# klasmodin/quflow

Hardware: AMD Instinct MI355X
Metric: isospectral timesteps/sec at N=1024 (1 GPU) + ensemble steps/sec at 1/2/4/8 GPUs (higher is better)
Workload: dtype f64

## Files before the change

### quflow_amd/csrc/api_context.hip

```cpp
#include <cmath>
#include <cstdarg>
#include <cstdio>
#include <cstdlib>
#include <cstring>
#include <limits>
#include <chrono>

#include "qf_api.h"

static thread_local char g_err[512] = "";

void qf_set_error(const char *fmt, ...)
{
    va_list ap;
    va_start(ap, fmt);
    vsnprintf(g_err, sizeof(g_err), fmt, ap);
    va_end(ap);
}

extern "C" {

int qf_version(void) { return QF_VERSION; }

int qf_device_info(int device, char *buf, int n)
// ... 93 lines not shown
    }
    QF_HIP(hipSetDevice(device));
    qf_ctx *ctx = new qf_ctx();
    ctx->N = N;
    ctx->device = device;
    if (const char *g = getenv("QUFLOW_HIP_GEMM")) {
        ctx->gemm_i8_allowed = (g[0] == 'i');
        if (g[0] == 'i' && strstr(g, "x6")) ctx->oz_digits = 6;
        if (g[0] == 'i' && strstr(g, "x65")) ctx->oz_digits2 = 5;
        if (g[0] == 'i' && strchr(g, 'h')) ctx->gemm_i8_hybrid = true;
        if (g[0] == 'i' && strchr(g, 'f') && !ctx->gemm_i8_hybrid) ctx->gemm_i8_first = true;
        if (g[0] == 'a') {
            ctx->gemm_i8_allowed = true;
            ctx->oz_digits = 6;
            ctx->oz_digits2 = 5;
            ctx->gemm_i8_min_n = 1024;
        }
    }
    if (const char *g = getenv("QUFLOW_HIP_GEMM2")) ctx->gemm_tri_allowed = !(g[0] == 'f');
    if (const char *g = getenv("QUFLOW_HIP_FUSED")) ctx->fused_allowed = !(g[0] == '0');
    if (const char *g = getenv("QUFLOW_HIP_I8_MIN_N")) ctx->gemm_i8_min_n = atoi(g);
    if (const char *g = getenv("QUFLOW_HIP_TRI_MIN_N")) ctx->gemm_tri_min_n = atoi(g);
    if (const char *g = getenv("QUFLOW_HIP_DEFER")) ctx->defer_allowed = !(g[0] == '0');
    if (getenv("QUFLOW_HIP_DEBUG"))
        if (const char *g = getenv("QUFLOW_HIP_DEBUG_DROP_FLAG")) ctx->debug_drop = atoi(g);
    if (const char *g = getenv("QUFLOW_HIP_FACTOR_CACHE_MB")) ctx->factor_budget_bytes = (size_t)(atoi(g) > 0 ? atoi(g) : 1) << 20;
    const size_t NN = (size_t)N * N;
    const size_t mbytes = NN * sizeof(cplx);
    int rc = QF_OK;
    auto fail = [&](int code) {
        qf_ctx_destroy(ctx);
        return code;
    };
#define QF_CREATE_HIP(call)                                                                   \
    do {                                                                                      \
        hipError_t _e = (call);                                                               \
        if (_e != hipSuccess) {                                                               \
            qf_set_error("%s failed: %s", #call, hipGetErrorString(_e));                     \
            return fail(QF_ERR_HIP);                                                          \
        }                                                                                     \
    } while (0)
    QF_CREATE_HIP(hipStreamCreateWithFlags(&ctx->stream, hipStreamNonBlocking));
    cplx **mats[] = {&ctx->W, &ctx->dW[0], &ctx->dW[1], &ctx->Whalf, &ctx->Phalf, &ctx->PW, &ctx->stage};
    for (cplx **m : mats) {
        QF_CREATE_HIP(hipMalloc((void **)m, mbytes));
        QF_CREATE_HIP(hipMemsetAsync(*m, 0, mbytes, ctx->stream));
// ... 226 lines not shown
{
    QF_TRY(check_ctx(ctx));
    QF_HIP(hipEventRecord(ctx->timer_start, ctx->stream));
    return QF_OK;
}

int qf_timer_stop(qf_ctx *ctx, double *elapsed_ms)
{
    QF_TRY(check_ctx(ctx));
    QF_HIP(hipEventRecord(ctx->timer_stop, ctx->stream));
    QF_HIP(hipEventSynchronize(ctx->timer_stop));
    float ms = 0.f;
    QF_HIP(hipEventElapsedTime(&ms, ctx->timer_start, ctx->timer_stop));
    if (elapsed_ms) *elapsed_ms = (double)ms;
    return QF_OK;
}

int qf_download_buffer(qf_ctx *ctx, int which, void *host)
{
    QF_TRY(check_ctx(ctx));
    const cplx *src = nullptr;
    switch (which) {
        case QF_BUF_W: src = ctx->W; break;
        case QF_BUF_DW: src = ctx->dW[ctx->dw_cur]; break;
        case QF_BUF_WHALF: src = ctx->Whalf; break;
        case QF_BUF_PHALF: src = ctx->Phalf; break;
        case QF_BUF_PW: src = ctx->PW; break;
        default:
            qf_set_error("qf_download_buffer: unknown buffer %d", which);
            return QF_ERR_INVALID;
    }
    if (!host) {
        qf_set_error("qf_download_buffer: null host pointer");
        return QF_ERR_INVALID;
    }
    QF_HIP(hipMemcpyAsync(host, src, (size_t)ctx->N * ctx->N * sizeof(cplx), hipMemcpyDeviceToHost, ctx->stream));
    QF_HIP(hipStreamSynchronize(ctx->stream));
    return QF_OK;
}

int qf_debug_modulus(qf_ctx *ctx, int n, const double *er_host, const double *ei_host, double *out_modulus_host,
                     double *out_sqrt_host)
{
    QF_TRY(check_ctx(ctx));
    if (n < 1 || (size_t)n > (size_t)ctx->N * ctx->N || !er_host || !ei_host || !out_modulus_host || !out_sqrt_host) {
        qf_set_error("qf_debug_modulus: bad arguments (n=%d)", n);
        return QF_ERR_INVALID;
// ... 14 lines not shown
```

### quflow_amd/csrc/api_isomp.hip

```cpp
#include <cmath>
#include <cstdarg>
#include <cstdio>
#include <cstdlib>
#include <cstring>
#include <limits>
#include <chrono>
#include <type_traits>
#include <utility>

#include "qf_api.h"

namespace {

#ifndef QF_RUN_AHEAD
#define QF_RUN_AHEAD 3
#endif

template <class S> constexpr bool is_c64 = std::is_same<S, qf_c64>::value;

template <class S> S *ws(qf_ctx *ctx)
{
    if constexpr (is_c64<S>) return ctx->c64;
    else return ctx;
}
// ... 87 lines not shown
    ctx->gemm_i8 = want_i8 && skew;
    ctx->gemm_tri32 = want_tri32 && skew && (!ctx->gemm_i8 || ctx->gemm_i8_first);
    if (ctx->gemm_tri32) QF_TRY(tri32_alloc(ctx));
    return QF_OK;
}

int select_second_product_c64(qf_ctx *ctx)
{
    qf_c64 *f = ctx->c64;
    f->tri = false;
    if (f->tri_allowed && ctx->gemm_tri_allowed && (qf_c64_tile(ctx) == 32 || ctx->N % 64 == 0) && ctx->N >= 64) {
        QF_TRY(check_skew(ctx, f));
        if (f->w_skew_known) {
            QF_TRY(qf_c64_tri_alloc(ctx));
            f->tri = true;
        }
    }
    return QF_OK;
}

bool triangle_product(const qf_ctx *ctx) { return (ctx->gemm_tri || ctx->gemm_tri32) && (!ctx->gemm_i8 || ctx->gemm_i8_first); }
bool triangle_product(const qf_c64 *f) { return f->tri; }

template <class S> int begin_increment(qf_ctx *ctx, S *w, bool carry)
{
    const size_t mbytes = (size_t)ctx->N * ctx->N * sizeof(*w->W);
    if (carry) {
        if (w->dw_cur != 0)
            QF_HIP(hipMemcpyAsync(w->dW[0], w->dW[w->dw_cur], mbytes, hipMemcpyDeviceToDevice, ctx->stream));
        QF_TRY(qf_launch_lincomb(ctx, 1, w->W, 1, w->dW[0], 0, w->Whalf));
    } else {
        QF_HIP(hipMemsetAsync(w->dW[0], 0, mbytes, ctx->stream));
        QF_HIP(hipMemcpyAsync(w->Whalf, w->W, mbytes, hipMemcpyDeviceToDevice, ctx->stream));
    }
    return QF_OK;
}

template <class S> int enqueue_iterations(qf_ctx *ctx, int step, int first, int count, double vareps)
{
    S *w = ws<S>(ctx);
    for (int i = first; i < first + count; ++i) {
        qf_guard g;
        g.state = ctx->state;
        g.step = step;
        g.iter = i;
        {
            prof_scope p(ctx, QF_KERNEL_POISSON);
            QF_TRY(launch_solve(ctx, w->Whalf, w->Phalf, vareps, g));
        }
        {
            prof_scope p(ctx, QF_KERNEL_GEMM1);
            QF_TRY(launch_gemm(ctx, w->Phalf, w->Whalf, w->PW, nullptr, g));
        }
        {
// ... 119 lines not shown
            const qf_epilogue ep = epilogue_of(ctx, true);
            QF_TRY(qf_launch_zgemm(ctx, ctx->PW, ctx->Phalf, nullptr, &ep, g));
            continue;
        }
        {
            prof_scope p(ctx, QF_KERNEL_SLICE);
            qf_oz_jobs jobs;
            jobs.n = 1;
            jobs.j[0].X = ctx->PW;
            jobs.j[0].planes = ctx->oz_planes[3];
            jobs.j[0].scale = ctx->oz_scale[3];
            QF_TRY(qf_launch_oz_slice(ctx, jobs, g, ctx->oz_digits2));
        }
        {
            prof_scope p(ctx, QF_KERNEL_GEMM2);
            const qf_epilogue ep = epilogue_of(ctx, true);
            QF_TRY(qf_launch_oz_gemm(ctx, ctx->oz_planes[3], ctx->oz_scale[3], ctx->oz_planes[0], ctx->oz_scale[0], nullptr,
                                     &ep, g, ctx->oz_digits2, ctx->oz_digits2 ? ctx->oz_digits : 0));
        }
    }
    return QF_OK;
}

template <class S> struct fused_run {
    qf_ctx *ctx = nullptr;
    int steps = 0, minit = 1, maxit = 1;
    double vareps = 0.0;
    int pred = 1, pred0 = 1;
    std::vector<int> enq_iters;
    int known = 0, enq = 0;
    bool first_seen = false;
    bool aborted = false;
    unsigned long long idle_polls = 0;

    int enqueue(int step, int first, int count)
    {
        if constexpr (!is_c64<S>)
            if (ctx->gemm_i8) return enqueue_iterations_fused_i8(ctx, step, first, count, vareps);
        return enqueue_iterations_fused<S>(ctx, step, first, count, vareps, step == steps - 1);
    }
    bool cold_start = true;
    void begin(qf_ctx *c, int steps_, int minit_, int maxit_, double vareps_)
    {
        ctx = c;
        cold_start = ws<S>(c)->increment_is_zero;
        steps = steps_;
        minit = minit_;
        maxit = maxit_;
        vareps = vareps_;
        pred = ctx->pred_iters;
        if (pred < minit) pred = minit;
        if (pred > maxit) pred = maxit;
        pred0 = ctx->pred_first_iters > 0 ? ctx->pred_first_iters : pred + 1;
        if (pred0 < pred) pred0 = pred;
        if (pred0 > maxit) pred0 = maxit;
        enq_iters.assign((size_t)steps + 1, 0);
        known = enq = 0;
        first_seen = false;
        aborted = false;
        idle_polls = 0;
    }
    bool done() const { return known >= steps; }
    int pump()
    {
        if (done()) return QF_OK;
        while (enq < steps && enq - known < QF_RUN_AHEAD) {
            const int n = (enq == 0 && cold_start) ? pred0 : pred;
            QF_TRY(enqueue(enq, 0, n));
            enq_iters[enq] = n;
            ++enq;
        }
        volatile qf_host_record *rec = ctx->host_rec;
        unsigned long long p = __atomic_load_n(&rec->progress, __ATOMIC_ACQUIRE);
        int ps = (int)(p >> 32), pi = (int)(p & 0xffffffffull);
        if (ps >= QF_STEP_ABORTED) {
            aborted = true;
            known = steps;
            return QF_OK;
        }
        if (!(ps > known || (ps == known && pi >= enq_iters[known]))) {
            if (++idle_polls > (1ull << 22)) {
                QF_HIP(hipStreamSynchronize(ctx->stream));
                p = __atomic_load_n(&rec->progress, __ATOMIC_ACQUIRE);
                ps = (int)(p >> 32);
                pi = (int)(p & 0xffffffffull);
                if (ps >= QF_STEP_ABORTED) {
                    aborted = true;
                    known = steps;
                    return QF_OK;
                }
                if (!(ps > known || (ps == known && pi >= enq_iters[known]))) {
                    qf_set_error("qf_isomp: device progress stuck at step %d iteration %d (waiting for step %d)", ps, pi, known);
                    return QF_ERR_STATE;
                }
            } else {
                return QF_OK;
            }
        }
        idle_polls = 0;
        if (ps > known) {
            const int it = rec->last_step_iters;
            if (known == 0 && ps == 1 && !first_seen && cold_start) {
                first_seen = true;
                if (it >= minit && it <= maxit) ctx->pred_first_iters = it;
            } else if (it >= minit && it <= maxit) {
                pred = it;
            }
            known = ps < enq ? ps : enq;
            if (done()) ctx->pred_iters = pred;
            return QF_OK;
        }
        const int have = enq_iters[known];
        if (have >= maxit) {
            qf_set_error("qf_isomp: step %d did not close after maxit=%d iterations (internal error)", known, maxit);
            return QF_ERR_STATE;
        }
        QF_TRY(enqueue(known, have, maxit - have));
        enq_iters[known] = maxit;
        enq = known + 1;
        if (pred < maxit) pred += 1;
        return QF_OK;
    }
};

bool poll_yields()
{
    static const int mode = [] {
        const char *e = getenv("QUFLOW_HIP_POLL");
        return (e && strcmp(e, "yield") == 0) ? 1 : 0;
    }();
    return mode == 1;
}

inline void poll_relax()
{
    if (poll_yields()) {
        sched_yield();
        return;
    }
#if defined(__x86_64__)
    __builtin_ia32_pause();
#endif
// ... 57 lines not shown
        QF_HIP(hipMemsetAsync(ctx->t32_arrive, 0, nt * (nt + 1) / 2 * sizeof(unsigned), ctx->stream));
    }
    if (ctx->c64 && ctx->c64->tri_arrive)
        QF_HIP(hipMemsetAsync(ctx->c64->tri_arrive, 0, ctx->c64->tri_arrive_count * sizeof(unsigned), ctx->stream));
    ctx->needs_reset = false;
    return QF_OK;
}

template <class S> int fused_enter(qf_ctx *ctx, double dt, double tol, int minit, int maxit, bool carry)
{
    S *w = ws<S>(ctx);
    const size_t mbytes = (size_t)ctx->N * ctx->N * sizeof(*w->W);
    const bool tol_on_device = tol < 0;
    const double tol_factor = tol_on_device ? mach_eps<S>(true) * dt / qf_hbar(ctx->N) : 0.0;
    QF_TRY(reset_after_abort(ctx));
    if constexpr (is_c64<S>) {
        QF_TRY(select_second_product_c64(ctx));
    } else {
        QF_TRY(select_second_product(ctx));
        ctx->defer = ctx->defer_allowed && !ctx->gemm_i8 && ctx->gemm_tri32 && ctx->N <= 512;
    }
    w->increment_is_zero = !carry;
    w->increment_valid = true;
    volatile qf_host_record *rec = ctx->host_rec;
    rec->progress = 0ull;
    rec->step_index = 0;
    rec->fault = 0;
    rec->nonfinite = 0;
    __atomic_thread_fence(__ATOMIC_SEQ_CST);
    if (is_c64<S> || carry) {
        if (tol_on_device) QF_TRY(qf_launch_norm_inf(ctx, w->W, ctx->scalars));
        QF_TRY(begin_increment(ctx, w, carry));
        QF_TRY(qf_launch_state_init(ctx, tol, minit, maxit, tol_on_device ? ctx->scalars : nullptr, tol_factor));
    } else {
        QF_TRY(qf_launch_call_begin(ctx, tol, minit, maxit, tol_on_device ? 1 : 0, tol_factor));
    }
    if (!w->W2) QF_HIP(hipMalloc((void **)&w->W2, mbytes));
    if (!w->Whalf2) QF_HIP(hipMalloc((void **)&w->Whalf2, mbytes));
    if constexpr (!is_c64<S>)
        if (ctx->gemm_i8) QF_TRY(qf_oz_alloc(ctx));
    return QF_OK;
}

template <class S> int fused_leave(qf_ctx *ctx, int steps, qf_isomp_stats *stats_out)
{
    S *w = ws<S>(ctx);
    volatile qf_host_record *rec = ctx->host_rec;
    const int w_parity = steps > 0 ? rec->w_parity : 0, wh_sel = steps > 0 ? rec->wh_sel : 0;
    w->dw_cur = steps > 0 ? rec->dw_parity : 0;
    if (w_parity) std::swap(w->W, w->W2);
    if (wh_sel) std::swap(w->Whalf, w->Whalf2);
    if (triangle_product(w) && steps > 0) {
        QF_TRY(qf_launch_mirror_lower(ctx, w->W));
        QF_TRY(qf_launch_mirror_lower(ctx, w->dW[w->dw_cur]));
    }
    if constexpr (!is_c64<S>)
        if (ctx->diag_at_exit) {
            QF_TRY(qf_enqueue_diagnostics(ctx));
            ctx->diag_valid = true;
        }
    QF_HIP(hipStreamSynchronize(ctx->stream));
    if (rec->nonfinite) {
        qf_set_error("array must not contain infs or NaNs");
        ctx->needs_reset = true;
        w->increment_valid = false;
        ctx->diag_valid = false;
        rec->nonfinite = 0;
        return QF_ERR_NONFINITE;
    }
    if (steps > 0 && rec->step_index != steps) {
        qf_set_error("qf_isomp: device completed %d of %d steps (internal error)", rec->step_index, steps);
        return QF_ERR_STATE;
    }
    if (rec->fault) {
        qf_set_error("qf_isomp: a device-side wait of the second product ran out (a parked partial tile or a mirrored result tile was never published)");
        return QF_ERR_STATE;
    }
    if (stats_out) {
        stats_out->total_iterations = steps > 0 ? rec->total_iterations : 0;
        stats_out->number_of_maxit = steps > 0 ? rec->number_of_maxit : 0;
        stats_out->tol_used = rec->tol;
        stats_out->last_resnorm = rec->resnorm;
    }
    return QF_OK;
}

void fused_abort(qf_ctx *ctx)
{
    (void)hipStreamSynchronize(ctx->stream);
    ctx->needs_reset = true;
    ctx->increment_valid = false;
    ctx->w_skew_known = false;
    if (ctx->c64) {
        ctx->c64->w_skew_known = false;
        ctx->c64->increment_valid = false;
    }
    ctx->host_rec->fault = 0;
    ctx->host_rec->nonfinite = 0;
}
// ... 262 lines not shown
    QF_HIP(hipMemcpyAsync(f->stage, W_host, bytes, hipMemcpyHostToDevice, ctx->stream));
    QF_HIP(hipMemcpyAsync(f->dW[0], dW_old_host, bytes, hipMemcpyHostToDevice, ctx->stream));
    QF_TRY(qf_launch_cgemm(ctx, f->Phalf, f->Whalf, f->PW, nullptr));
    qf_epilogue_f ep = epilogue_of(f, false);
    ep.W = f->stage;
    if (tri) {
        QF_TRY(qf_launch_cgemm_tri(ctx, f->PW, f->Phalf, &ep));
        QF_TRY(qf_launch_mirror_lower(ctx, f->dW[1]));
        QF_TRY(qf_launch_sum_rowpart(ctx, f->rowpart, (N + qf_c64_tile(ctx) - 1) / qf_c64_tile(ctx), ctx->rowsum));
    } else {
        QF_TRY(qf_launch_cgemm(ctx, f->PW, f->Phalf, nullptr, &ep));
        QF_TRY(qf_launch_sum_rowpart(ctx, f->rowpart, f->rowpart_tiles, ctx->rowsum));
    }
    QF_HIP(hipMemcpyAsync(dW_new_host, f->dW[1], bytes, hipMemcpyDeviceToHost, ctx->stream));
    QF_HIP(hipMemcpyAsync(Whalf_new_host, f->Whalf, bytes, hipMemcpyDeviceToHost, ctx->stream));
    QF_HIP(hipMemcpyAsync(rowsum_host, ctx->rowsum, (size_t)N * sizeof(double), hipMemcpyDeviceToHost, ctx->stream));
    QF_HIP(hipStreamSynchronize(ctx->stream));
    return QF_OK;
}

}

int qf_rowpart_slots(const qf_ctx *ctx) { return ctx->gemm_tri ? ctx->N / 64 : ctx->gemm_tri32 ? (ctx->N + 31) / 32 : ctx->rowpart_tiles; }

int qf_enqueue_diagnostics(qf_ctx *ctx)
{
    QF_TRY(qf_launch_solve(ctx, ctx->poisson, ctx->W, ctx->stage, 1.0, 1));
    QF_TRY(qf_launch_inner2(ctx, ctx->W, ctx->stage, ctx->scalars + 2));
    QF_HIP(hipMemcpyAsync(ctx->host_scalars, ctx->scalars + 2, 2 * sizeof(double), hipMemcpyDeviceToHost, ctx->stream));
    return QF_OK;
}

int qf_isomp_multi(qf_ctx **ctxs, int k, double dt, int steps, double tol, int minit, int maxit, qf_isomp_stats *stats_out)
{
    return isomp_multi<qf_ctx>(ctxs, k, dt, steps, tol, minit, maxit, stats_out);
}

int qf_c64_isomp_multi(qf_ctx **ctxs, int k, double dt, int steps, double tol, int minit, int maxit, qf_isomp_stats *stats_out)
{
    return isomp_multi<qf_c64>(ctxs, k, dt, steps, tol, minit, maxit, stats_out);
}

int qf_isomp(qf_ctx *ctx, double dt, int steps, double tol, int minit, int maxit, int compsum,
             int reinitialize, qf_isomp_stats *stats_out)
{
    return isomp_impl<qf_ctx>(ctx, dt, steps, tol, minit, maxit, compsum, reinitialize, stats_out, false);
// ... 132 lines not shown
```

### quflow_amd/csrc/elementwise.hip

```cpp
#include "qf_internal.h"

#pragma clang fp contract(off)

namespace {

constexpr int TU = 32;

__device__ __forceinline__ cplx make_c(double re, double im) { return make_double2(re, im); }
__device__ __forceinline__ float2 make_c(float re, float im) { return make_float2(re, im); }
__device__ __forceinline__ double modulus_d(cplx z) { return hypot(z.x, z.y); }
__device__ __forceinline__ double modulus_d(float2 z) { return (double)hypotf(z.x, z.y); }
__device__ __forceinline__ double re_dot_d(cplx a, cplx b) { return a.x * b.x + a.y * b.y; }
__device__ __forceinline__ double re_dot_d(float2 a, float2 b) { return (double)(a.x * b.x + a.y * b.y); }

__device__ void qf_step_advance(qf_dev_state *state, qf_host_record *rec, const qf_guard &guard)
{
    const bool mine = state->step_index == guard.step;
    const bool complete = mine && (state->step_done != 0 || state->iters_this_step >= state->maxit);
    int incomplete = 0;
    if (complete) {
        if (!state->step_done) state->number_of_maxit += 1;
        rec->last_step_iters = state->iters_this_step;
        state->step_index += 1;
        state->iters_this_step = 0;
// ... 145 lines not shown
}

__global__ __launch_bounds__(256) void k_neg_conj_transpose(int N, const cplx *__restrict__ X, cplx *__restrict__ out)
{
    __shared__ cplx Ts[TU][TU + 1];
    const int tx = threadIdx.x & 31, ty = threadIdx.x >> 5;
    const int i0 = blockIdx.y * TU, j0 = blockIdx.x * TU;
    for (int r = ty; r < TU; r += 8) {
        const int gj = j0 + r, gi = i0 + tx;
        cplx tv = make_double2(0.0, 0.0);
        if (gj < N && gi < N) tv = X[(size_t)gj * N + gi];
        Ts[r][tx] = tv;
    }
    __syncthreads();
    for (int r = ty; r < TU; r += 8) {
        const int gi = i0 + r, gj = j0 + tx;
        if (gi < N && gj < N) {
            const cplx t = Ts[tx][r];
            out[(size_t)gi * N + gj] = make_double2(-t.x, t.y);
        }
    }
}

template <class C>
__global__ __launch_bounds__(256) void k_mirror_lower(int N, C *__restrict__ X)
{
    using R = typename C::value_type;
    __shared__ C Ts[TU][TU + 1];
    const int tx = threadIdx.x & 31, ty = threadIdx.x >> 5;
    const int bi = blockIdx.y, bj = blockIdx.x;
    if (bj > bi) return;
    const int i0 = bi * TU, j0 = bj * TU;
    for (int r = ty; r < TU; r += 8) {
        const int gj = j0 + r, gi = i0 + tx;
        C tv = make_c(R(0), R(0));
        if (gj < N && gi < N) tv = X[(size_t)gj * N + gi];
        Ts[r][tx] = tv;
    }
    __syncthreads();
    for (int r = ty; r < TU; r += 8) {
        const int gi = i0 + r, gj = j0 + tx;
        if (gi < N && gj < N && gj < gi) {
            const C t = Ts[tx][r];
            X[(size_t)gi * N + gj] = make_c(-t.x, t.y);
        }
    }
}

__global__ __launch_bounds__(256) void k_magnetic_fix(int N, const cplx *__restrict__ BTP, const cplx *__restrict__ BT,
                                                       cplx *__restrict__ dW, const cplx *__restrict__ dW_old,
                                                       const cplx *__restrict__ W, cplx *__restrict__ Whalf,
                                                       double *__restrict__ rowpart)
{
    __shared__ cplx Tp[TU][TU + 1], Tb[TU][TU + 1];
    __shared__ double rs[8][TU];
    const int tx = threadIdx.x & 31, ty = threadIdx.x >> 5;
    const int i0 = blockIdx.y * TU, j0 = blockIdx.x * TU;
    for (int r = ty; r < TU; r += 8) {
        const int gj = j0 + r, gi = i0 + tx;
        cplx a = make_double2(0.0, 0.0), b = a;
        if (gj < N && gi < N) {
            a = BTP[(size_t)gj * N + gi];
            b = BT[(size_t)gj * N + gi];
        }
        Tp[r][tx] = a;
        Tb[r][tx] = b;
    }
    __syncthreads();
    for (int r = ty; r < TU; r += 8) {
// ... 343 lines not shown
__global__ __launch_bounds__(256) void k_inner_partial(size_t n, const cplx *__restrict__ A,
                                                        const cplx *__restrict__ B, double *__restrict__ partial)
{
    __shared__ double part[4];
    double s = 0.0;
    for (size_t e = (size_t)blockIdx.x * 256 + threadIdx.x; e < n; e += (size_t)gridDim.x * 256) {
        cplx a = A[e], b = B[e];
        s += a.x * b.x + a.y * b.y;
    }
    s = wave_sum(s);
    if ((threadIdx.x & 63) == 0) part[threadIdx.x >> 6] = s;
    __syncthreads();
    if (threadIdx.x == 0) partial[blockIdx.x] = (part[0] + part[1]) + (part[2] + part[3]);
}

__global__ __launch_bounds__(64) void k_sum_partials(int n, const double *__restrict__ partial, double *__restrict__ out)
{
    double s = 0.0;
    for (int i = threadIdx.x; i < n; i += 64) s += partial[i];
    s = wave_sum(s);
    if (threadIdx.x == 0) out[0] = s;
}

template <class C>
__global__ __launch_bounds__(256) void k_inner2(size_t n, const C *__restrict__ A, const C *__restrict__ B,
                                                 double *__restrict__ partial, unsigned *ticket, double *__restrict__ out)
{
    using R = typename C::value_type;
    __shared__ double pab[4], paa[4];
    __shared__ int last;
    double sab = 0.0, saa = 0.0;
    const size_t stride = (size_t)gridDim.x * 256;
    for (size_t e0 = (size_t)blockIdx.x * 256 + threadIdx.x; e0 < n; e0 += 4 * stride) {
        C a[4], b[4];
#pragma unroll
        for (int u = 0; u < 4; ++u) {
            const size_t e = e0 + u * stride;
            a[u] = b[u] = make_c(R(0), R(0));
            if (e < n) {
                a[u] = A[e];
                b[u] = B[e];
            }
        }
#pragma unroll
        for (int u = 0; u < 4; ++u) {
            if (e0 + u * stride < n) {
                sab += re_dot_d(a[u], b[u]);
                saa += re_dot_d(a[u], a[u]);
            }
// ... 1 lines not shown
    }
    sab = wave_sum(sab);
    saa = wave_sum(saa);
    if ((threadIdx.x & 63) == 0) {
        pab[threadIdx.x >> 6] = sab;
        paa[threadIdx.x >> 6] = saa;
    }
    __syncthreads();
    if (threadIdx.x == 0) {
        __hip_atomic_store(partial + blockIdx.x, (pab[0] + pab[1]) + (pab[2] + pab[3]), __ATOMIC_RELAXED, __HIP_MEMORY_SCOPE_AGENT);
        __hip_atomic_store(partial + 1024 + blockIdx.x, (paa[0] + paa[1]) + (paa[2] + paa[3]), __ATOMIC_RELAXED, __HIP_MEMORY_SCOPE_AGENT);
        last = last_block_of_launch(ticket, blockIdx.x, gridDim.x) ? 1 : 0;
    }
    __syncthreads();
    if (!last || threadIdx.x >= 64) return;
    double s0 = 0.0, s1 = 0.0;
    for (int i = threadIdx.x; i < (int)gridDim.x; i += 64) {
        s0 += __hip_atomic_load(partial + i, __ATOMIC_RELAXED, __HIP_MEMORY_SCOPE_AGENT);
        s1 += __hip_atomic_load(partial + 1024 + i, __ATOMIC_RELAXED, __HIP_MEMORY_SCOPE_AGENT);
    }
    s0 = wave_sum(s0);
    s1 = wave_sum(s1);
    if (threadIdx.x == 0) {
        out[0] = s0;
        out[1] = s1;
    }
}

__global__ __launch_bounds__(256) void k_mhd_sums(int N, const cplx *__restrict__ W, const cplx *__restrict__ P,
                                                   const cplx *__restrict__ Theta, double *__restrict__ partial, unsigned *ticket,
                                                   double *__restrict__ out)
{
    __shared__ double part[5][4];
    __shared__ int last;
    const unsigned n = (unsigned)N * (unsigned)N;
    double s[5] = {0.0, 0.0, 0.0, 0.0, 0.0};
    const unsigned stride = gridDim.x * 256u;
    for (unsigned e = blockIdx.x * 256u + threadIdx.x; e < n; e += stride) {
        const int i = (int)(e / (unsigned)N), j = (int)(e - (unsigned)i * (unsigned)N);
        const cplx w = W[e], p = P[e], t = Theta[e];
        const cplx lt = qf_laplace_entry<double, cplx>(N, Theta, i, j);
        s[0] += re_dot_d(w, p);
        s[1] += re_dot_d(t, lt);
        s[2] += re_dot_d(w, t);
        s[3] += re_dot_d(t, t);
        s[4] += re_dot_d(w, w);
    }
#pragma unroll
    for (int q = 0; q < 5; ++q) {
        s[q] = wave_sum(s[q]);
// ... 28 lines not shown
    hipLaunchKernelGGL(k_mhd_sums, dim3(blocks), dim3(256), 0, ctx->stream, ctx->N, W, P, Theta, part, ctx->ticket + 640, out_dev);
    QF_HIP(hipGetLastError());
    return QF_OK;
}

int qf_launch_call_begin(qf_ctx *ctx, double tol, int minit, int maxit, int auto_tol, double tol_factor)
{
    hipLaunchKernelGGL(k_call_begin, dim3(ctx->N < 1024 ? ctx->N : 1024), dim3(256), 0, ctx->stream, ctx->N, ctx->W, ctx->dW[0], ctx->Whalf, ctx->rowsum,
                       ctx->ticket + 600, ctx->state, ctx->host_rec, tol, minit, maxit, auto_tol, tol_factor);
    QF_HIP(hipGetLastError());
    return QF_OK;
}

template <class C> int qf_launch_inner2(qf_ctx *ctx, const C *A, const C *B, double *out_dev)
{
    const size_t n = (size_t)ctx->N * ctx->N;
    int blocks = (int)((n + 255) / 256);
    if (blocks > 1024) blocks = 1024;
    hipLaunchKernelGGL(k_inner2<C>, dim3(blocks), dim3(256), 0, ctx->stream, n, A, B, ctx->scalars + 64, ctx->ticket + 640, out_dev);
    QF_HIP(hipGetLastError());
    return QF_OK;
}

template <class C>
int qf_launch_update(qf_ctx *ctx, const C *PW, C *W, const C *dW_a, const C *dW_b, C *Whalf, qf_same<C> *kahan_c,
                     int reinitialize, qf_guard guard)
{
    const int N = ctx->N;
    dim3 grid((N + TU - 1) / TU, (N + TU - 1) / TU), block(256);
    C *a = const_cast<C *>(dW_a), *b = const_cast<C *>(dW_b);
    if (kahan_c)
        hipLaunchKernelGGL((k_update<C, true>), grid, block, 0, ctx->stream, N, PW, W, a, b, Whalf, kahan_c, reinitialize, guard,
                           guard.state ? ctx->state : nullptr, ctx->host_rec, ctx->ticket);
    else
        hipLaunchKernelGGL((k_update<C, false>), grid, block, 0, ctx->stream, N, PW, W, a, b, Whalf, kahan_c, reinitialize, guard,
                           guard.state ? ctx->state : nullptr, ctx->host_rec, ctx->ticket);
    QF_HIP(hipGetLastError());
    return QF_OK;
}

int qf_launch_norm_decide(qf_ctx *ctx, const double *rowpart, int tiles, qf_guard guard)
{
    hipLaunchKernelGGL(k_norm_decide, dim3(1), dim3(1024), 0, ctx->stream, ctx->N, tiles, rowpart, ctx->state, guard);
    QF_HIP(hipGetLastError());
    return QF_OK;
}
// ... 57 lines not shown
    return QF_OK;
}

template <class C>
int qf_launch_lincomb(qf_ctx *ctx, double a, const C *X, double b, const qf_same<C> *Y, double c, C *out)
{
    using R = typename C::value_type;
    const size_t n = (size_t)ctx->N * ctx->N;
    int blocks = (int)((n + 255) / 256);
    if (blocks > 4096) blocks = 4096;
    hipLaunchKernelGGL(k_lincomb<C>, dim3(blocks), dim3(256), 0, ctx->stream, ctx->N, (R)a, X, (R)b, Y, (R)c, out);
    QF_HIP(hipGetLastError());
    return QF_OK;
}

template <class C> int qf_launch_mirror_lower(qf_ctx *ctx, C *X)
{
    const int tiles = (ctx->N + TU - 1) / TU;
    hipLaunchKernelGGL(k_mirror_lower<C>, dim3(tiles, tiles), dim3(256), 0, ctx->stream, ctx->N, X);
    QF_HIP(hipGetLastError());
    return QF_OK;
}

int qf_launch_neg_conj_transpose(qf_ctx *ctx, const cplx *X, cplx *out)
{
    const int N = ctx->N;
    dim3 grid((N + TU - 1) / TU, (N + TU - 1) / TU), block(256);
    hipLaunchKernelGGL(k_neg_conj_transpose, grid, block, 0, ctx->stream, N, X, out);
    QF_HIP(hipGetLastError());
    return QF_OK;
}

int qf_launch_sum_rowpart(qf_ctx *ctx, const double *rowpart, int tiles, double *rowsum_dev)
{
    hipLaunchKernelGGL(k_sum_rowpart, dim3((ctx->N + 255) / 256), dim3(256), 0, ctx->stream, ctx->N, tiles, rowpart,
                       rowsum_dev);
    QF_HIP(hipGetLastError());
    return QF_OK;
}

template <class C> int qf_launch_skew_defect(qf_ctx *ctx, const C *A, double *out_dev)
{
    const int N = ctx->N;
    int blocks = N < 1024 ? N : 1024;
    double *partial = ctx->scalars + 64;
    hipLaunchKernelGGL(k_skew_defect_partial<C>, dim3(blocks), dim3(256), 0, ctx->stream, N, A, partial, partial + 1024);
    QF_HIP(hipGetLastError());
    hipLaunchKernelGGL(k_max_partials2, dim3(1), dim3(64), 0, ctx->stream, blocks, partial, partial + 1024, out_dev);
    QF_HIP(hipGetLastError());
    return QF_OK;
}

template int qf_launch_update(qf_ctx *, const cplx *, cplx *, const cplx *, const cplx *, cplx *, cplx *, int, qf_guard);
template int qf_launch_update(qf_ctx *, const float2 *, float2 *, const float2 *, const float2 *, float2 *, float2 *, int, qf_guard);
template int qf_launch_mirror_lower(qf_ctx *, cplx *);
template int qf_launch_mirror_lower(qf_ctx *, float2 *);
template int qf_launch_norm_inf(qf_ctx *, const cplx *, double *);
template int qf_launch_norm_inf(qf_ctx *, const float2 *, double *);
template int qf_launch_inner2(qf_ctx *, const cplx *, const cplx *, double *);
template int qf_launch_inner2(qf_ctx *, const float2 *, const float2 *, double *);
template int qf_launch_skew_defect(qf_ctx *, const cplx *, double *);
template int qf_launch_skew_defect(qf_ctx *, const float2 *, double *);
template int qf_launch_lincomb(qf_ctx *, double, const cplx *, double, const cplx *, double, cplx *);
template int qf_launch_lincomb(qf_ctx *, double, const float2 *, double, const float2 *, double, float2 *);

int qf_launch_inner(qf_ctx *ctx, const cplx *A, const cplx *B, double *out_dev)
{
    const size_t n = (size_t)ctx->N * ctx->N;
    int blocks = (int)((n + 255) / 256);
    if (blocks > 1024) blocks = 1024;
    double *partial = ctx->scalars + 64;
    hipLaunchKernelGGL(k_inner_partial, dim3(blocks), dim3(256), 0, ctx->stream, n, A, B, partial);
    QF_HIP(hipGetLastError());
    hipLaunchKernelGGL(k_sum_partials, dim3(1), dim3(64), 0, ctx->stream, blocks, partial, out_dev);
    QF_HIP(hipGetLastError());
    return QF_OK;
}

__global__ void k_debug_modulus(int n, const double *__restrict__ er, const double *__restrict__ ei, double *__restrict__ out_mod,
// ... 15 lines not shown
```

### quflow_amd/csrc/qf_api.h

```cpp
#pragma once

#include "qf_internal.h"

#include <sched.h>

namespace {
int drain_events(qf_ctx *ctx);

struct prof_scope {
    qf_ctx *ctx;
    qf_event_pair ev;
    bool active;
    prof_scope(qf_ctx *c, int id) : ctx(c), active(((c->profile_mask >> id) & 1) != 0)
    {
        ctx->plan_role = id;
        if (!active) return;
        if ((ctx->prof_seen[id]++ % ctx->profile_stride) != 0) {
            active = false;
            return;
        }
        if (ctx->events_free.empty()) {
            if (hipEventCreate(&ev.start) != hipSuccess || hipEventCreate(&ev.stop) != hipSuccess) {
                active = false;
                return;
// ... 41 lines not shown
{
    if (!ctx) {
        qf_set_error("null qf_ctx");
        return QF_ERR_INVALID;
    }
    QF_HIP(hipSetDevice(ctx->device));
    return QF_OK;
}

int read_scalar(qf_ctx *ctx, const double *dev, double *out)
{
    QF_HIP(hipMemcpyAsync(ctx->host_scalars, dev, sizeof(double), hipMemcpyDeviceToHost, ctx->stream));
    QF_HIP(hipStreamSynchronize(ctx->stream));
    *out = ctx->host_scalars[0];
    return QF_OK;
}

}

extern "C" {
int qf_need_c64(qf_ctx *ctx);
int qf_oz_alloc(qf_ctx *ctx);
int qf_rowpart_slots(const qf_ctx *ctx);
int qf_enqueue_diagnostics(qf_ctx *ctx);
}
```

### quflow_amd/csrc/qf_internal.h

```cpp
#pragma once

#include <hip/hip_runtime.h>

#include <atomic>
#include <cstdarg>
#include <cstdio>
#include <map>
#include <mutex>
#include <string>
#include <vector>

#include "../../include/quflow_hip.h"

typedef double2 cplx;

hipError_t qf_guard_malloc(void **p, size_t bytes);
hipError_t qf_guard_free(void *p);
#define hipMalloc(p, n) qf_guard_malloc((void **)(p), (n))
#define hipFree(p) qf_guard_free((void *)(p))

void qf_set_error(const char *fmt, ...);
struct qf_ctx;
inline void qf_plan_note(qf_ctx *ctx, unsigned long long key, const char *fmt, ...) __attribute__((format(printf, 3, 4)));

// ... 32 lines not shown
    int minit, maxit;
    int dw_parity;
    int fault;
    int w_parity;
    int wh_sel;
    int pending;
    int pending_iter;
};


struct qf_host_record {
    unsigned long long seq;
    long long total_iterations;
    long long number_of_maxit;
    double resnorm;
    int step_index;
    int last_step_iters;
    int incomplete;
    int nonfinite;
    unsigned long long progress;
    double tol;
    int w_parity, wh_sel, dw_parity;
    int fault;
};

struct qf_decide {
    const double *rowpart = nullptr;
    int slots = 0;
    qf_dev_state *state_rw = nullptr;
    qf_host_record *rec = nullptr;
    unsigned *ticket = nullptr;
};

struct qf_guard {
    const qf_dev_state *state = nullptr;
    int step = 0;
    int iter = 0;
    const void *alt = nullptr;
};

#ifdef __HIPCC__
__device__ __forceinline__ bool qf_guard_iter(const qf_guard &g)
{
    if (!g.state) return true;
    return g.state->step_index == g.step && g.state->step_done == 0 && g.state->iters_this_step == g.iter;
}
__device__ __forceinline__ bool qf_guard_step_end(const qf_guard &g)
{
    if (!g.state) return true;
    return g.state->step_index == g.step && (g.state->step_done != 0 || g.state->iters_this_step >= g.state->maxit);
}
template <int CTRL> __device__ __forceinline__ double qf_dpp_f64(double v)
{
    const int lo = __builtin_amdgcn_update_dpp(0, __double2loint(v), CTRL, 0xf, 0xf, true);
    const int hi = __builtin_amdgcn_update_dpp(0, __double2hiint(v), CTRL, 0xf, 0xf, true);
    return __hiloint2double(hi, lo);
}
__device__ __forceinline__ double qf_row16_sum(double v)
{
    v += qf_dpp_f64<0xB1>(v);
    v += qf_dpp_f64<0x4E>(v);
    v += qf_dpp_f64<0x141>(v);
    v += qf_dpp_f64<0x140>(v);
    return v;
}

__device__ __forceinline__ double qf_modulus(double er, double ei)
{
    const double x = er * er + ei * ei;
    const double y = __builtin_amdgcn_rsq(x);
    double g = x * y, h = 0.5 * y;
    const double r = __builtin_fma(-h, g, 0.5);
    g = __builtin_fma(g, r, g);
// ... 39 lines not shown
        wr += a * q.x;
        wi += a * q.y;
    }
    C2 o;
    o.x = wr;
    o.y = wi;
    return o;
}
#endif

struct qf_c64 {
    float2 *W = nullptr;
    float2 *dW[2] = {nullptr, nullptr};
    float2 *Whalf = nullptr, *Phalf = nullptr, *PW = nullptr;
    float2 *kahan_c = nullptr;
    float2 *stage = nullptr;
    float *lap = nullptr;
    float2 *tab = nullptr;
    double *rowpart = nullptr;
    int rowpart_tiles = 0;
    int dw_cur = 0;
    bool increment_is_zero = true;
    bool increment_valid = false;
    float2 *W2 = nullptr, *Whalf2 = nullptr;
    float2 *tri_partial = nullptr;
    unsigned *tri_arrive = nullptr;
    size_t tri_arrive_count = 0;
    int tri_split = 2, tri_split_diag = 2;
    bool tri_allowed = true, tri = false, w_skew_known = false;
};
struct qf_ctri {
    float2 *partial = nullptr;
    unsigned *arrive = nullptr;
    int split = 2, split_diag = 2;
};
struct qf_smem_attr {
    std::atomic<size_t> bytes[64] = {};
};
inline std::mutex &qf_smem_attr_mutex()
{
    static std::mutex m;
    return m;
}
inline int qf_smem_attr_set(qf_smem_attr &a, const void *fn, int device, size_t bytes)
{
    const int d = device & 63;
// ... 49 lines not shown
    int *perm = nullptr;
    unsigned long long *word = nullptr;
};

struct qf_geom_ws {
    cplx *R[2] = {nullptr, nullptr};
    cplx *grad = nullptr;
    hipEvent_t ev[3] = {nullptr, nullptr, nullptr};
    bool timed = false;
};

struct qf_ctx {
    int N = 0;
    int device = 0;
    hipStream_t stream = nullptr;

    cplx *W = nullptr;
    bool w_skew_known = false;
    cplx *dW[2] = {nullptr, nullptr};
    int dw_cur = 0;
    bool increment_is_zero = true;
    int pred_first_iters = 0;
    bool increment_valid = false;
    cplx *W2 = nullptr;
    cplx *Whalf2 = nullptr;
    bool fused_allowed = true;
    cplx *Whalf = nullptr;
    cplx *Phalf = nullptr;
    cplx *PW = nullptr;
    cplx *kahan_c = nullptr;
    cplx *stage = nullptr;
    signed char *oz_planes[4] = {nullptr, nullptr, nullptr, nullptr};
    double *oz_scale[4] = {nullptr, nullptr, nullptr, nullptr};
    bool gemm_i8 = false;
    bool gemm_i8_allowed = false;
    bool gemm_i8_hybrid = false;
    bool gemm_i8_first = false;
    int gemm_i8_min_n = 768;
    int oz_digits = 5;
    int oz_digits2 = 0;
    cplx *oz_tbuf = nullptr;
    unsigned *oz_tflags = nullptr;
    unsigned oz_epoch = 0;
    double *oz_diag = nullptr;
    std::vector<cplx *> multi;
    double *multi_rowpart = nullptr;
// ... 25 lines not shown
    unsigned long long forcing_key = 0, forcing_fp = 0;
    bool forcing_on = false, forcing_f0_on = false;
    double forcing_aW = 0.0, forcing_aP = 0.0, forcing_alap = 0.0;

    double *basis = nullptr;
    cplx *sh_stage = nullptr;
    double *sh_omega = nullptr;
    long long sh_shr_count = 0;
    long long slab_budget = 0;
    double *slab = nullptr;
    size_t slab_cap = 0;
    qf_sht sht;
    qf_eigh_ws eigh;
    qf_geom_ws geom;

    double *rowpart = nullptr;
    int rowpart_tiles = 0;
    double *rowsum = nullptr;
    double *scalars = nullptr;
    double *host_scalars = nullptr;
    qf_dev_state *state = nullptr;
    qf_host_record *host_rec = nullptr;
    bool diag_at_exit = false, diag_valid = false;
    unsigned *ticket = nullptr;
    int pred_iters = 3;
    bool gemm_tri_allowed = true;
    bool gemm_tri = false;
    int gemm_tri_min_n = 960;
    bool gemm_tri32 = false;
    int tri32_split = 2, tri32_split_diag = 1;
    cplx *t32_partial = nullptr;
    unsigned *t32_arrive = nullptr;
    bool defer_allowed = true;
    bool defer = false;
    int num_cus = 0;
    cplx *sk_partial = nullptr;
    unsigned *sk_flags = nullptr;
    int sk_slots = 0;
    unsigned sk_epoch = 0;
    int sk_epi_units = 0;
    int sk_epi_units_fused = 2;
    int sk_min_units = 8;
    int debug_drop = 0;
    bool needs_reset = false;

    qf_c64 *c64 = nullptr;
// ... 167 lines not shown
template <class T> using qf_same = typename qf_same_type<T>::type;
template <class C>
int qf_launch_update(qf_ctx *ctx, const C *PW, C *W, const C *dW_a, const C *dW_b, C *Whalf, qf_same<C> *kahan_c,
                     int reinitialize, qf_guard guard = qf_guard());
int qf_launch_debug_modulus(qf_ctx *ctx, int n, const double *er, const double *ei, double *out_mod, double *out_sqrt);
int qf_launch_norm_from_rowpart(qf_ctx *ctx, const double *rowpart, int tiles, double *out_dev);
int qf_launch_fold_nonfinite(qf_ctx *ctx, const double *in_dev, double *acc_dev);
int qf_launch_norm_decide(qf_ctx *ctx, const double *rowpart, int tiles, qf_guard guard);
int qf_launch_state_init(qf_ctx *ctx, double tol, int minit, int maxit, const double *norm_dev = nullptr, double tol_factor = 0.0);
template <class C> int qf_launch_norm_inf(qf_ctx *ctx, const C *A, double *out_dev);
int qf_launch_call_begin(qf_ctx *ctx, double tol, int minit, int maxit, int auto_tol, double tol_factor);
template <class C> int qf_launch_inner2(qf_ctx *ctx, const C *A, const C *B, double *out_dev);
int qf_launch_inner(qf_ctx *ctx, const cplx *A, const cplx *B, double *out_dev);
int qf_launch_mhd_sums(qf_ctx *ctx, const cplx *W, const cplx *P, const cplx *Theta, double *part, double *out_dev);
int qf_launch_erk_stage(qf_ctx *ctx, const cplx *A, const cplx *B, double inv_hb, const cplx *W, cplx *acc,
                        double c_acc, cplx *Wp, double c_wp, cplx *Wout, double c_fin);
int qf_launch_magnetic_fix(qf_ctx *ctx, const cplx *BTP, const cplx *BT, cplx *dW, const cplx *dW_old, const cplx *W,
                           cplx *Whalf, double *rowpart);
int qf_launch_magnetic_update(qf_ctx *ctx, const cplx *BT, cplx *W, const cplx *dW, cplx *Whalf);
template <class C>
int qf_launch_lincomb(qf_ctx *ctx, double a, const C *X, double b, const qf_same<C> *Y, double c, C *out);
int qf_launch_neg_conj_transpose(qf_ctx *ctx, const cplx *X, cplx *out);
template <class C> int qf_launch_mirror_lower(qf_ctx *ctx, C *X);
int qf_launch_sum_rowpart(qf_ctx *ctx, const double *rowpart, int tiles, double *rowsum_dev);
template <class C> int qf_launch_skew_defect(qf_ctx *ctx, const C *A, double *out_dev);
```

Before: 2700.

## Enqueue call-end mirror and diagnostics on device ahead of host sync; defer increment mirror

At the end of a fused isospectral call, the mirror of W's lower triangle and the exit diagnostics (Poisson solve plus inner products) are now queued speculatively on the stream as soon as the last step is enqueued. They are guarded to run only when the device state confirms the call end, and the diagnostics are written straight into the host-mapped record. The lower-triangle mirror of the increment dW is deferred until it is actually needed (next carry or download). This removes the host-side launches and an extra mirror kernel after the synchronisation, at the cost of extra guard-checking kernels and more state bookkeeping.

```diff
diff --git a/quflow_amd/csrc/api_context.hip b/quflow_amd/csrc/api_context.hip
--- a/quflow_amd/csrc/api_context.hip
+++ b/quflow_amd/csrc/api_context.hip
@@ -139,6 +139,7 @@
     if (const char *g = getenv("QUFLOW_HIP_I8_MIN_N")) ctx->gemm_i8_min_n = atoi(g);
     if (const char *g = getenv("QUFLOW_HIP_TRI_MIN_N")) ctx->gemm_tri_min_n = atoi(g);
     if (const char *g = getenv("QUFLOW_HIP_DEFER")) ctx->defer_allowed = !(g[0] == '0');
+    if (const char *g = getenv("QUFLOW_HIP_CALL_END")) ctx->call_end_device = !(g[0] == 'h');
     if (getenv("QUFLOW_HIP_DEBUG"))
         if (const char *g = getenv("QUFLOW_HIP_DEBUG_DROP_FLAG")) ctx->debug_drop = atoi(g);
     if (const char *g = getenv("QUFLOW_HIP_FACTOR_CACHE_MB")) ctx->factor_budget_bytes = (size_t)(atoi(g) > 0 ? atoi(g) : 1) << 20;
@@ -411,7 +412,10 @@
     const cplx *src = nullptr;
     switch (which) {
         case QF_BUF_W: src = ctx->W; break;
-        case QF_BUF_DW: src = ctx->dW[ctx->dw_cur]; break;
+        case QF_BUF_DW:
+            QF_TRY(qf_restore_increment(ctx));
+            src = ctx->dW[ctx->dw_cur];
+            break;
         case QF_BUF_WHALF: src = ctx->Whalf; break;
         case QF_BUF_PHALF: src = ctx->Phalf; break;
         case QF_BUF_PW: src = ctx->PW; break;
diff --git a/quflow_amd/csrc/api_isomp.hip b/quflow_amd/csrc/api_isomp.hip
--- a/quflow_amd/csrc/api_isomp.hip
+++ b/quflow_amd/csrc/api_isomp.hip
@@ -133,14 +133,24 @@
 bool triangle_product(const qf_ctx *ctx) { return (ctx->gemm_tri || ctx->gemm_tri32) && (!ctx->gemm_i8 || ctx->gemm_i8_first); }
 bool triangle_product(const qf_c64 *f) { return f->tri; }
 
+template <class S> int restore_increment(qf_ctx *ctx, S *w)
+{
+    if (!w->dw_lower_stale) return QF_OK;
+    QF_TRY(qf_launch_mirror_lower(ctx, w->dW[w->dw_cur]));
+    w->dw_lower_stale = false;
+    return QF_OK;
+}
+
 template <class S> int begin_increment(qf_ctx *ctx, S *w, bool carry)
 {
     const size_t mbytes = (size_t)ctx->N * ctx->N * sizeof(*w->W);
     if (carry) {
+        QF_TRY(restore_increment(ctx, w));
         if (w->dw_cur != 0)
             QF_HIP(hipMemcpyAsync(w->dW[0], w->dW[w->dw_cur], mbytes, hipMemcpyDeviceToDevice, ctx->stream));
         QF_TRY(qf_launch_lincomb(ctx, 1, w->W, 1, w->dW[0], 0, w->Whalf));
     } else {
+        w->dw_lower_stale = false;
         QF_HIP(hipMemsetAsync(w->dW[0], 0, mbytes, ctx->stream));
         QF_HIP(hipMemcpyAsync(w->Whalf, w->W, mbytes, hipMemcpyDeviceToDevice, ctx->stream));
     }
@@ -306,6 +316,22 @@
     return QF_OK;
 }
 
+template <class S> int enqueue_call_end(qf_ctx *ctx, int steps)
+{
+    S *w = ws<S>(ctx);
+    qf_guard g;
+    g.state = ctx->state;
+    g.step = steps;
+    g.iter = 0;
+    if (triangle_product(w) && steps > 0) QF_TRY(qf_launch_mirror_lower_due(ctx, w->W, w->W2, g));
+    if constexpr (!is_c64<S>)
+        if (ctx->diag_at_exit) {
+            QF_TRY(qf_launch_solve(ctx, ctx->poisson, (steps & 1) ? ctx->W2 : ctx->W, ctx->stage, 1.0, 1, g));
+            QF_TRY(qf_launch_inner2_due(ctx, ctx->W, ctx->W2, ctx->stage, g));
+        }
+    return QF_OK;
+}
+
 template <class S> struct fused_run {
     qf_ctx *ctx = nullptr;
     int steps = 0, minit = 1, maxit = 1;
@@ -315,6 +341,7 @@
     int known = 0, enq = 0;
     bool first_seen = false;
     bool aborted = false;
+    bool end_enq = false;
     unsigned long long idle_polls = 0;
 
     int enqueue(int step, int first, int count)
@@ -342,6 +369,8 @@
         known = enq = 0;
         first_seen = false;
         aborted = false;
+        end_enq = false;
+        ctx->call_end_queued = false;
         idle_polls = 0;
     }
     bool done() const { return known >= steps; }
@@ -353,6 +382,10 @@
             QF_TRY(enqueue(enq, 0, n));
             enq_iters[enq] = n;
             ++enq;
+        }
+        if (ctx->call_end_device && enq == steps && !end_enq) {
+            QF_TRY(enqueue_call_end<S>(ctx, steps));
+            end_enq = true;
         }
         volatile qf_host_record *rec = ctx->host_rec;
         unsigned long long p = __atomic_load_n(&rec->progress, __ATOMIC_ACQUIRE);
@@ -391,7 +424,10 @@
                 pred = it;
             }
             known = ps < enq ? ps : enq;
-            if (done()) ctx->pred_iters = pred;
+            if (done()) {
+                ctx->pred_iters = pred;
+                ctx->call_end_queued = end_enq;
+            }
             return QF_OK;
         }
         const int have = enq_iters[known];
@@ -402,6 +438,7 @@
         QF_TRY(enqueue(known, have, maxit - have));
         enq_iters[known] = maxit;
         enq = known + 1;
+        end_enq = false;
         if (pred < maxit) pred += 1;
         return QF_OK;
     }
@@ -505,6 +542,8 @@
     }
     w->increment_is_zero = !carry;
     w->increment_valid = true;
+    if (!carry) w->dw_lower_stale = false;
+    ctx->call_end_queued = false;
     volatile qf_host_record *rec = ctx->host_rec;
     rec->progress = 0ull;
     rec->step_index = 0;
@@ -530,15 +569,25 @@
     S *w = ws<S>(ctx);
     volatile qf_host_record *rec = ctx->host_rec;
     const int w_parity = steps > 0 ? rec->w_parity : 0, wh_sel = steps > 0 ? rec->wh_sel : 0;
+    const bool closed_early = steps > 0 && rec->nonfinite != 0;
+    const bool by_tag = ctx->call_end_device && !closed_early;
+    bool diag_in_record = false;
+    if (by_tag) {
+        if (!ctx->call_end_queued) QF_TRY(enqueue_call_end<S>(ctx, steps));
+        if constexpr (!is_c64<S>)
+            if (ctx->diag_at_exit) diag_in_record = true;
+    }
+    ctx->call_end_queued = false;
     w->dw_cur = steps > 0 ? rec->dw_parity : 0;
     if (w_parity) std::swap(w->W, w->W2);
     if (wh_sel) std::swap(w->Whalf, w->Whalf2);
     if (triangle_product(w) && steps > 0) {
-        QF_TRY(qf_launch_mirror_lower(ctx, w->W));
-        QF_TRY(qf_launch_mirror_lower(ctx, w->dW[w->dw_cur]));
+        if (!by_tag) QF_TRY(qf_launch_mirror_lower(ctx, w->W));
+        w->dw_lower_stale = true;
+        if (!ctx->call_end_device) QF_TRY(restore_increment(ctx, w));
     }
     if constexpr (!is_c64<S>)
-        if (ctx->diag_at_exit) {
+        if (ctx->diag_at_exit && !by_tag) {
             QF_TRY(qf_enqueue_diagnostics(ctx));
             ctx->diag_valid = true;
         }
@@ -558,6 +607,11 @@
     if (rec->fault) {
         qf_set_error("qf_isomp: a device-side wait of the second product ran out (a parked partial tile or a mirrored result tile was never published)");
         return QF_ERR_STATE;
+    }
+    if (diag_in_record) {
+        ctx->host_scalars[0] = rec->diag[0];
+        ctx->host_scalars[1] = rec->diag[1];
+        ctx->diag_valid = true;
     }
     if (stats_out) {
         stats_out->total_iterations = steps > 0 ? rec->total_iterations : 0;
@@ -866,6 +920,8 @@
 }
 
 int qf_rowpart_slots(const qf_ctx *ctx) { return ctx->gemm_tri ? ctx->N / 64 : ctx->gemm_tri32 ? (ctx->N + 31) / 32 : ctx->rowpart_tiles; }
+
+int qf_restore_increment(qf_ctx *ctx) { return restore_increment(ctx, ctx); }
 
 int qf_enqueue_diagnostics(qf_ctx *ctx)
 {
diff --git a/quflow_amd/csrc/elementwise.hip b/quflow_amd/csrc/elementwise.hip
--- a/quflow_amd/csrc/elementwise.hip
+++ b/quflow_amd/csrc/elementwise.hip
@@ -191,8 +191,7 @@
     }
 }
 
-template <class C>
-__global__ __launch_bounds__(256) void k_mirror_lower(int N, C *__restrict__ X)
+template <class C> __device__ __forceinline__ void mirror_lower_tile(int N, C *__restrict__ X)
 {
     using R = typename C::value_type;
     __shared__ C Ts[TU][TU + 1];
@@ -214,6 +213,19 @@
             X[(size_t)gi * N + gj] = make_c(-t.x, t.y);
         }
     }
+}
+
+template <class C>
+__global__ __launch_bounds__(256) void k_mirror_lower(int N, C *__restrict__ X)
+{
+    mirror_lower_tile(N, X);
+}
+
+template <class C>
+__global__ __launch_bounds__(256) void k_mirror_lower_due(int N, C *W0, C *W1, qf_guard guard)
+{
+    if (!qf_guard_call_end(guard)) return;
+    mirror_lower_tile(N, guard.state->w_parity ? W1 : W0);
 }
 
 __global__ __launch_bounds__(256) void k_magnetic_fix(int N, const cplx *__restrict__ BTP, const cplx *__restrict__ BT,
@@ -603,9 +615,9 @@
     if (threadIdx.x == 0) out[0] = s;
 }
 
-template <class C>
-__global__ __launch_bounds__(256) void k_inner2(size_t n, const C *__restrict__ A, const C *__restrict__ B,
-                                                 double *__restrict__ partial, unsigned *ticket, double *__restrict__ out)
+template <class C, bool TO_HOST>
+__device__ __forceinline__ void inner2_body(size_t n, const C *__restrict__ A, const C *__restrict__ B,
+                                            double *__restrict__ partial, unsigned *ticket, double *__restrict__ out)
 {
     using R = typename C::value_type;
     __shared__ double pab[4], paa[4];
@@ -653,10 +665,31 @@
     s0 = wave_sum(s0);
     s1 = wave_sum(s1);
     if (threadIdx.x == 0) {
-        out[0] = s0;
-        out[1] = s1;
-    }
-}
+        if constexpr (TO_HOST) {
+            __hip_atomic_store(out, s0, __ATOMIC_RELAXED, __HIP_MEMORY_SCOPE_SYSTEM);
+            __hip_atomic_store(out + 1, s1, __ATOMIC_RELEASE, __HIP_MEMORY_SCOPE_SYSTEM);
+        } else {
+            out[0] = s0;
+            out[1] = s1;
+        }
+    }
+}
+
+template <class C>
+__global__ __launch_bounds__(256) void k_inner2(size_t n, const C *__restrict__ A, const C *__restrict__ B,
+                                                 double *__restrict__ partial, unsigned *ticket, double *__restrict__ out)
+{
+    inner2_body<C, false>(n, A, B, partial, ticket, out);
+}
+
+__global__ __launch_bounds__(256) void k_inner2_due(size_t n, const cplx *W0, const cplx *W1, const cplx *__restrict__ B,
+                                                     double *__restrict__ partial, unsigned *ticket, qf_host_record *rec,
+                                                     qf_guard guard)
+{
+    if (!qf_guard_call_end(guard)) return;
+    inner2_body<cplx, true>(n, guard.state->w_parity ? W1 : W0, B, partial, ticket, rec->diag);
+}
+
 
 __global__ __launch_bounds__(256) void k_mhd_sums(int N, const cplx *__restrict__ W, const cplx *__restrict__ P,
                                                    const cplx *__restrict__ Theta, double *__restrict__ partial, unsigned *ticket,
@@ -731,6 +764,17 @@
     return QF_OK;
 }
 
+int qf_launch_inner2_due(qf_ctx *ctx, const cplx *W0, const cplx *W1, const cplx *B, qf_guard guard)
+{
+    const size_t n = (size_t)ctx->N * ctx->N;
+    int blocks = (int)((n + 255) / 256);
+    if (blocks > 1024) blocks = 1024;
+    hipLaunchKernelGGL(k_inner2_due, dim3(blocks), dim3(256), 0, ctx->stream, n, W0, W1, B, ctx->scalars + 64, ctx->ticket + 640,
+                       ctx->host_rec, guard);
+    QF_HIP(hipGetLastError());
+    return QF_OK;
+}
+
 template <class C>
 int qf_launch_update(qf_ctx *ctx, const C *PW, C *W, const C *dW_a, const C *dW_b, C *Whalf, qf_same<C> *kahan_c,
                      int reinitialize, qf_guard guard)
@@ -834,6 +878,14 @@
     return QF_OK;
 }
 
+template <class C> int qf_launch_mirror_lower_due(qf_ctx *ctx, C *W0, C *W1, qf_guard guard)
+{
+    const int tiles = (ctx->N + TU - 1) / TU;
+    hipLaunchKernelGGL(k_mirror_lower_due<C>, dim3(tiles, tiles), dim3(256), 0, ctx->stream, ctx->N, W0, W1, guard);
+    QF_HIP(hipGetLastError());
+    return QF_OK;
+}
+
 int qf_launch_neg_conj_transpose(qf_ctx *ctx, const cplx *X, cplx *out)
 {
     const int N = ctx->N;
@@ -867,6 +919,8 @@
 template int qf_launch_update(qf_ctx *, const float2 *, float2 *, const float2 *, const float2 *, float2 *, float2 *, int, qf_guard);
 template int qf_launch_mirror_lower(qf_ctx *, cplx *);
 template int qf_launch_mirror_lower(qf_ctx *, float2 *);
+template int qf_launch_mirror_lower_due(qf_ctx *, cplx *, cplx *, qf_guard);
+template int qf_launch_mirror_lower_due(qf_ctx *, float2 *, float2 *, qf_guard);
 template int qf_launch_norm_inf(qf_ctx *, const cplx *, double *);
 template int qf_launch_norm_inf(qf_ctx *, const float2 *, double *);
 template int qf_launch_inner2(qf_ctx *, const cplx *, const cplx *, double *);
diff --git a/quflow_amd/csrc/qf_api.h b/quflow_amd/csrc/qf_api.h
--- a/quflow_amd/csrc/qf_api.h
+++ b/quflow_amd/csrc/qf_api.h
@@ -87,5 +87,6 @@
 int qf_need_c64(qf_ctx *ctx);
 int qf_oz_alloc(qf_ctx *ctx);
 int qf_rowpart_slots(const qf_ctx *ctx);
+int qf_restore_increment(qf_ctx *ctx);
 int qf_enqueue_diagnostics(qf_ctx *ctx);
 }
diff --git a/quflow_amd/csrc/qf_internal.h b/quflow_amd/csrc/qf_internal.h
--- a/quflow_amd/csrc/qf_internal.h
+++ b/quflow_amd/csrc/qf_internal.h
@@ -78,6 +78,7 @@
     double tol;
     int w_parity, wh_sel, dw_parity;
     int fault;
+    double diag[2];
 };
 
 struct qf_decide {
@@ -105,6 +106,11 @@
 {
     if (!g.state) return true;
     return g.state->step_index == g.step && (g.state->step_done != 0 || g.state->iters_this_step >= g.state->maxit);
+}
+__device__ __forceinline__ bool qf_guard_call_end(const qf_guard &g)
+{
+    if (!g.state) return true;
+    return g.state->step_index == g.step;
 }
 template <int CTRL> __device__ __forceinline__ double qf_dpp_f64(double v)
 {
@@ -190,6 +196,7 @@
     int dw_cur = 0;
     bool increment_is_zero = true;
     bool increment_valid = false;
+    bool dw_lower_stale = false;
     float2 *W2 = nullptr, *Whalf2 = nullptr;
     float2 *tri_partial = nullptr;
     unsigned *tri_arrive = nullptr;
@@ -285,6 +292,7 @@
     bool increment_is_zero = true;
     int pred_first_iters = 0;
     bool increment_valid = false;
+    bool dw_lower_stale = false;
     cplx *W2 = nullptr;
     cplx *Whalf2 = nullptr;
     bool fused_allowed = true;
@@ -356,6 +364,7 @@
     qf_dev_state *state = nullptr;
     qf_host_record *host_rec = nullptr;
     bool diag_at_exit = false, diag_valid = false;
+    bool call_end_device = true, call_end_queued = false;
     unsigned *ticket = nullptr;
     int pred_iters = 3;
     bool gemm_tri_allowed = true;
@@ -569,5 +578,7 @@
 int qf_launch_lincomb(qf_ctx *ctx, double a, const C *X, double b, const qf_same<C> *Y, double c, C *out);
 int qf_launch_neg_conj_transpose(qf_ctx *ctx, const cplx *X, cplx *out);
 template <class C> int qf_launch_mirror_lower(qf_ctx *ctx, C *X);
+template <class C> int qf_launch_mirror_lower_due(qf_ctx *ctx, C *W0, C *W1, qf_guard guard);
+int qf_launch_inner2_due(qf_ctx *ctx, const cplx *W0, const cplx *W1, const cplx *B, qf_guard guard);
 int qf_launch_sum_rowpart(qf_ctx *ctx, const double *rowpart, int tiles, double *rowsum_dev);
 template <class C> int qf_launch_skew_defect(qf_ctx *ctx, const C *A, double *out_dev);
```

Result: no change. 2699 (-0.0%).
